# swap357/llama3.np

Measured on AMD Instinct MI355X. Metric: tokens/s stories15M batch-256 seq-256 prefill; % fp32 MFMA peak on FFN GEMM, higher is better.
Workload: dtype fp32; 1 GPU; stories15M prefill, B=256 per GPU x L=256, start_pos 0; global_batch=256, seq_len=256, parallelism=dp1 (batch rows) + RCCL logits gather

## Files before the change

include/llama3hip.h:

```cpp
#ifndef LLAMA3HIP_H
#define LLAMA3HIP_H

#include <stddef.h>
#include <stdint.h>

#ifdef __cplusplus
extern "C" {
#endif

typedef struct l3_ctx l3_ctx;

typedef struct l3_dims {
    int32_t dim;
    int32_t n_layers;
    int32_t n_heads;
    int32_t n_kv_heads;
    int32_t vocab_size;
    int32_t hidden_dim;
    int32_t max_seq_len;
    int32_t max_batch_size;
    float norm_eps;
} l3_dims;

enum l3_weight_kind {
// ... 2 lines not shown
    L3_W_K = 2,
    L3_W_V = 3,
    L3_W_O = 4,
    L3_W_GATE = 5,
    L3_W_UP = 6,
    L3_W_DOWN = 7,
    L3_W_ATTN_NORM = 8,
    L3_W_FFN_NORM = 9,
    L3_W_FINAL_NORM = 10,
    L3_W_LM_HEAD = 11
};

enum l3_kernel_id {
    L3_K_EMBED = 0, L3_K_QKV = 1, L3_K_ATTN = 2, L3_K_OPROJ = 3, L3_K_GATEUP = 4,
    L3_K_DOWN = 5, L3_K_LMHEAD = 6, L3_K_ARGMAX = 7, L3_K_GATHER = 8, L3_K_EMBED_QKV = 9,
    L3_K_FFN = 10, L3_K_COUNT = 11
};

const char* l3_last_error(void);
int l3_device_count(int32_t* n);
int l3_version(int32_t* major, int32_t* minor);
const char* l3_source_hash(void);

int l3_create(int32_t device, const l3_dims* dims, l3_ctx** out);
enum l3_kv_dtype { L3_KV_F32 = 0, L3_KV_BF16 = 1 };
int l3_create_kv(int32_t device, const l3_dims* dims, int32_t kv_dtype, l3_ctx** out);
int l3_kv_info(l3_ctx* ctx, int32_t* dtype, int64_t* bytes);
int l3_destroy(l3_ctx* ctx);
int l3_upload_weight(l3_ctx* ctx, int32_t layer, int32_t kind, const float* host,
                     int64_t rows, int64_t cols);
int l3_finalize(l3_ctx* ctx);
int l3_reset_cache(l3_ctx* ctx);

int l3_forward_host(l3_ctx* ctx, const int64_t* ids_host, int32_t B, int32_t L,
                    int32_t start_pos, float* logits_host);
int l3_set_batch_split(l3_ctx* ctx, int32_t parts, int64_t min_tokens);
int l3_set_last_layer_rows(l3_ctx* ctx, int32_t all_rows);
int l3_set_gemm_x6(l3_ctx* ctx, int32_t on);
int l3_set_weight_bf16(l3_ctx* ctx, int32_t mode);
int l3_weight_bf16_info(l3_ctx* ctx, int32_t* mode, int64_t* bytes, int64_t* gemv_launches);
int l3_set_weight_bf16_rows(l3_ctx* ctx, int32_t max_rows, int64_t min_bytes);
int l3_weight_bf16_rows_info(l3_ctx* ctx, int32_t* max_rows, int64_t* min_bytes, int64_t* launches);
int l3_set_weight_fp8(l3_ctx* ctx, int32_t mode);
int l3_weight_fp8_info(l3_ctx* ctx, int32_t* mode, int64_t* bytes, int64_t* gemv_launches,
                       int64_t* rows_launches);
int l3_set_embed_qkv(l3_ctx* ctx, int32_t on, int64_t max_bytes);
int l3_set_ffn_fused(l3_ctx* ctx, int32_t on);
int l3_forward_dev(l3_ctx* ctx, const int32_t* ids_dev, int32_t B, int32_t L,
                   int32_t start_pos, float* logits_dev);
int l3_score_host(l3_ctx* ctx, const int64_t* ids_host, const int64_t* targets_host, int32_t B, int32_t L,
                  int32_t start_pos, float* logprobs_host, int32_t* argmax_host);
int l3_set_score_workspace(l3_ctx* ctx, int64_t bytes);
int l3_set_sampling(l3_ctx* ctx, float temperature, int32_t top_k, float top_p, uint64_t seed);
int l3_get_sampling(l3_ctx* ctx, float* temperature, int32_t* top_k, float* top_p, uint64_t* seed);
int l3_sample_uniform(uint64_t seed, int32_t row, int32_t pos, float* u);

int l3_greedy_step_host(l3_ctx* ctx, const int64_t* ids_host, int32_t B, int32_t L,
                        int32_t start_pos, int64_t* next_ids_host, float* logits_host);

int l3_greedy_generate_host(l3_ctx* ctx, const int64_t* ids_host, int32_t B, int32_t L,
                            int32_t max_new_tokens, int64_t* out_ids_host);
// ... 225 lines not shown
```

llama3.np_amd/csrc/attention.hip:

```cpp
#include "attn_kernel.h"

namespace l3 {

static void report(AttnRoute* rt, int kernel, int HD, int QBW, int G, int KT, dim3 grid) {
    if (rt) *rt = AttnRoute{kernel, HD, QBW, G, KT, {(int)grid.x, (int)grid.y, (int)grid.z}};
}

template <int HD, int QBW, int G, int KT>
static hipError_t launch(const AttnArgs& a, hipStream_t s, AttnRoute* rt) {
    constexpr int QW = 16 * QBW * (4 / G);
    dim3 grid((a.L + QW - 1) / QW, a.H / G, a.B), block(256);
    report(rt, ATTN_PREFILL, HD, QBW, G, KT, grid);
    hipLaunchKernelGGL((attn_fwd_kernel<HD, QBW, G, KT, true>), grid, block, 0, s, a);
    return hipGetLastError();
}

template <int HD, int KT, int QBIG, int G>
static hipError_t launch_g(const AttnArgs& a, hipStream_t s, AttnRoute* rt) {
    constexpr int WPH = 4 / G;
    if (a.L <= 16 * WPH) return launch<HD, 1, G, KT>(a, s, rt);
    if (QBIG > 2 && a.L <= 32 * WPH) return launch<HD, 2, G, KT>(a, s, rt);
    return launch<HD, QBIG, G, KT>(a, s, rt);
}

template <int HD, int KT, int QBIG>
static hipError_t launch_hd(const AttnArgs& a, hipStream_t s, AttnRoute* rt) {
    const int n_rep = a.H / a.KVH;
    if (n_rep % 4 == 0) return launch_g<HD, KT, QBIG, 4>(a, s, rt);
    if (n_rep % 2 == 0) return launch_g<HD, KT, QBIG, 2>(a, s, rt);
    return launch_g<HD, KT, QBIG, 1>(a, s, rt);
}

template <int HD>
static hipError_t launch_decode(const AttnArgs& a, hipStream_t s, AttnRoute* rt) {
    constexpr int R = 256 / (HD / 4);
    const size_t lds = ((size_t)R * HD + a.Smax) * 4;
    if (a.wo) {
        if (!a.parts || a.D <= 0 || a.D % 4) return hipErrorInvalidValue;
        const dim3 grid(a.H, a.B, (a.D + 63) / 64);
        report(rt, ATTN_DECODE_OPROJ, HD, 0, 0, 0, grid);
        hipLaunchKernelGGL((attn_decode_kernel<HD, true>), grid, dim3(256), lds, s, a);
    } else {
        const dim3 grid(a.H, a.B);
        report(rt, ATTN_DECODE, HD, 0, 0, 0, grid);
        hipLaunchKernelGGL((attn_decode_kernel<HD, false>), grid, dim3(256), lds, s, a);
// ... 45 lines not shown
            case 128: return launch_decode<128>(a, s, rt);
            default: return hipErrorInvalidValue;
        }
    }
    switch (a.HD) {
        case 16: return launch_hd<16, 64, 4>(a, s, rt);
        case 32: return launch_hd<32, 64, 4>(a, s, rt);
        case 48: return launch_hd<48, 64, 4>(a, s, rt);
        case 64: return launch_hd<64, 64, 4>(a, s, rt);
        case 96: return launch_hd<96, 32, 1>(a, s, rt);
        case 128: return launch_hd<128, 32, 1>(a, s, rt);
        default: return hipErrorInvalidValue;
    }
}

hipError_t dcheck_collect_attention(unsigned* out) { return dcheck_collect(out); }

}
```

llama3.np_amd/csrc/attn_kernel.h:

```cpp
#pragma once
#include <type_traits>

#include "kernels.h"

namespace l3 {

typedef float f32x4 __attribute__((ext_vector_type(4)));

template <int HD, int QBW, int G, int KT, bool PK = false>
__global__ void __launch_bounds__(256, 2) attn_fwd_kernel(AttnArgs p) {
    static_assert(HD % 16 == 0 && KT % 16 == 0 && (G == 1 || G == 2 || G == 4), "shape");
    constexpr int WPH = 4 / G;
    constexpr int NQB = QBW * WPH;
    constexpr int QW = 16 * NQB;
    constexpr int ND = HD / 16;
    constexpr int KSTR = HD + 8;
    constexpr int VSTR = HD + 4;
    constexpr int K_F4 = KT * HD / 4;
    constexpr int K_IT = (K_F4 + 255) / 256;
    constexpr int KG = KT / 16;

    __shared__ __attribute__((aligned(16))) float Ks[2][KT][KSTR];
    __shared__ __attribute__((aligned(16))) float Vs[2][KT][VSTR];

// ... 5 lines not shown
    const int qdim = p.H * HD;
    const int fq = lane & 15;
    const int fk = 4 * (lane >> 4);

    int qblk[QBW];
#pragma unroll
    for (int j = 0; j < QBW; ++j)
        qblk[j] = (j & 1) ? (2 * WPH * (j >> 1) + 2 * WPH - 1 - part) : (2 * WPH * (j >> 1) + part);

    const int start_pos = start_of(p);
    const int q_lo = p.q_first + qt * QW;
    const int q_hi = min(p.L, q_lo + QW);
    const int key_end = start_pos + q_hi;
    const int ntiles = (key_end + KT - 1) / KT;
    if (threadIdx.x == 0) L3_DCHECK(start_pos >= 0 && start_pos + p.L <= p.Smax, CHK_ATTN_KEYS);

    f32x4 qreg[QBW][ND];
    f32x4 o[QBW][ND];
    float m_run[QBW], l_run[QBW];
#pragma unroll
    for (int j = 0; j < QBW; ++j) {
        const int ql = min(q_lo + qblk[j] * 16 + fq, p.L - 1);
        const float* src = p.q + ((int64_t)b * p.L + ql) * qdim + h * HD + fk;
#pragma unroll
        for (int dg = 0; dg < ND; ++dg) {
            qreg[j][dg] = *reinterpret_cast<const f32x4*>(src + dg * 16);
            o[j][dg] = f32x4{0.f, 0.f, 0.f, 0.f};
        }
        m_run[j] = -INFINITY;
        l_run[j] = 0.f;
    }

    const int64_t kv_base = ((int64_t)b * p.KVH + kvh) * p.Smax;
    f32x4 rk[K_IT], rv[K_IT];
    auto gload = [&](int tile) {
#pragma unroll
        for (int i = 0; i < K_IT; ++i) {
            const int f = tid + 256 * i;
            const int row = f / (HD / 4), c = (f % (HD / 4)) * 4;
            const int key = min(tile * KT + row, p.Smax - 1);
            if (K_F4 % 256 == 0 || f < K_F4) {
                rk[i] = *reinterpret_cast<const f32x4*>(p.cache_k + (kv_base + key) * HD + c);
                rv[i] = *reinterpret_cast<const f32x4*>(p.cache_v + (kv_base + key) * HD + c);
            }
        }
    };
    auto sstore = [&](int buf) {
#pragma unroll
        for (int i = 0; i < K_IT; ++i) {
            const int f = tid + 256 * i;
            if (K_F4 % 256 == 0 || f < K_F4) {
                const int row = f / (HD / 4), c = (f % (HD / 4)) * 4;
                *reinterpret_cast<f32x4*>(&Ks[buf][row][c]) = rk[i];
                *reinterpret_cast<f32x4*>(&Vs[buf][row][c]) = rv[i];
            }
        }
    };

    gload(0);
    sstore(0);
    __syncthreads();
    int cur = 0;
    for (int tile = 0; tile < ntiles; ++tile) {
        if (tile + 1 < ntiles) gload(tile + 1);
        const int k0 = tile * KT;
        auto qblock_tile = [&](const int j, const int qblock_first, const int qmax_abs, auto masked_tag) {
            constexpr bool MASKED = decltype(masked_tag)::value;
            const int q_abs = start_pos + qblock_first + fq;
            f32x4 sacc[KG];
            bool live[KG];
#pragma unroll
            for (int kg = 0; kg < KG; ++kg) {
                live[kg] = !MASKED || (k0 + kg * 16) <= qmax_abs;
                sacc[kg] = f32x4{0.f, 0.f, 0.f, 0.f};
            }
// ... 90 lines not shown
                }
                __builtin_amdgcn_sched_group_barrier(0x008, 2, 1);
            }
        };
#pragma unroll
        for (int j = 0; j < QBW; ++j) {
            const int qblock_first = q_lo + qblk[j] * 16;
            if (qblock_first >= p.L) continue;
            const int qmax_abs = start_pos + min(qblock_first + 15, p.L - 1);
            if (k0 > qmax_abs) continue;
            if (k0 + KT - 1 <= start_pos + qblock_first)
                qblock_tile(j, qblock_first, qmax_abs, std::integral_constant<bool, false>{});
            else
                qblock_tile(j, qblock_first, qmax_abs, std::integral_constant<bool, true>{});
        }
        if (tile + 1 < ntiles) sstore(cur ^ 1);
        __syncthreads();
        cur ^= 1;
    }

#pragma unroll
    for (int j = 0; j < QBW; ++j) {
        float l = l_run[j];
        l = sum_xor16_32(l);
        const int ql = q_lo + qblk[j] * 16 + fq;
        if (ql < p.L) {
            const float inv = 1.0f / l;
            float* dst = p.out + ((int64_t)b * p.L + ql) * qdim + h * HD + fk;
#pragma unroll
            for (int dg = 0; dg < ND; ++dg)
                *reinterpret_cast<f32x4*>(dst + dg * 16) = o[j][dg] * inv;
// ... 96 lines not shown
```

llama3.np_amd/csrc/embed_qkv.h:

```cpp
#pragma once
#include "gemm_kernel.h"

namespace l3 {

__device__ __forceinline__ f32x4 rope_rotate4(const f32x4 v, const float2 c, const float2 s) {
    return f32x4{__builtin_fmaf(v.x, c.x, -(v.y * s.x)), __builtin_fmaf(v.x, s.x, v.y * c.x),
                 __builtin_fmaf(v.z, c.y, -(v.w * s.y)), __builtin_fmaf(v.z, s.y, v.w * c.y)};
}

constexpr int EQ_ROWS = 16;
constexpr int EQ_R = 4;

template <int CPB>
__global__ void __launch_bounds__(256) embed_qkv_kernel(EmbedQkvArgs p) {
    static_assert(CPB == 64 || CPB == 128 || CPB == 256, "whole waves per row group");
    static_assert(EQ_ROWS % EQ_R == 0, "whole passes");
    constexpr int RPB = 256 / CPB;
    const int cq = threadIdx.x % CPB, rsub = threadIdx.x / CPB;
    const int qdim = p.H * p.HD, kvdim = p.KVH * p.HD, qkvn = qdim + 2 * kvdim, nq = qkvn >> 2;
    const int hd2 = p.HD >> 1;
    const int quad = blockIdx.y * CPB + cq;
    const bool active = quad < nq;
    const int col = 4 * min(quad, nq - 1);
    const int sec = col < qdim ? 0 : (col < qdim + kvdim ? 1 : 2);
// ... 48 lines not shown
```

llama3.np_amd/csrc/kernels.h:

```cpp
#pragma once
#include <hip/hip_runtime.h>
#include <stdint.h>
#include <stdlib.h>

namespace l3 {

inline int env_knob(const char* name, int def) {
    const char* e = getenv(name);
    return e && *e ? atoi(e) : def;
}

enum CheckClass : int { CHK_KV_SLOT = 0, CHK_ATTN_KEYS = 1, CHK_TOKEN_ID = 2, CHK_N = 4 };
#ifdef L3_DEVICE_CHECKS
static __device__ unsigned l3_dcheck_counts[CHK_N];
#define L3_DCHECK(cond, cls)                                                      \
    do {                                                                          \
        if (!(cond)) atomicAdd(&::l3::l3_dcheck_counts[(cls)], 1u);               \
    } while (0)
static inline hipError_t dcheck_collect(unsigned* out) {
    unsigned h[CHK_N] = {};
    hipError_t e = hipMemcpyFromSymbol(h, HIP_SYMBOL(l3_dcheck_counts), sizeof h, 0, hipMemcpyDeviceToHost);
    if (e != hipSuccess) return e;
    for (int i = 0; i < CHK_N; ++i) out[i] += h[i];
    const unsigned z[CHK_N] = {};
// ... 248 lines not shown
__device__ __forceinline__ const float* res_at(const GemmArgs& p, int64_t row, int col) {
    return res_row(p, row) + col;
}

struct AttnArgs {
    const float* q;
    int q_first;
    const float* cache_k;
    const float* cache_v;
    float* out;
    int B, L, start_pos, H, KVH, HD, Smax;
    const int* pos_dev;
    const float* wo;
    float* parts;
    int D;
};

template <typename Args>
__device__ __forceinline__ int start_of(const Args& p) {
    return p.pos_dev ? *p.pos_dev : p.start_pos;
}

struct RaggedState {
    int32_t* pos;
    int32_t* cur_id;
    int32_t* finished;
    int32_t* n_out;
    const int32_t* len;
    const int32_t* budget;
    int32_t* out;
// ... 147 lines not shown
};
bool ffn_fused_takes(int64_t M, int D, int FD);
hipError_t launch_ffn_fused(const FfnArgs& a, hipStream_t s);

struct EmbedQkvArgs {
    const float* table;
    const int32_t* ids;
    float* q_out;
    float* cache_k; float* cache_v;
    const float* rope_cos; const float* rope_sin;
    int T, L, start_pos, H, KVH, HD, Smax, VS;
};
hipError_t launch_qkv_table(const GemmArgs& a, hipStream_t s);
hipError_t launch_embed_qkv(const EmbedQkvArgs& a, hipStream_t s);
hipError_t launch_split_planes(const float* w, unsigned short* w3, int64_t rows, int K, hipStream_t s);
enum AttnRouteKernel : int { ATTN_NONE = -1, ATTN_PREFILL = 0, ATTN_DECODE = 1, ATTN_DECODE_OPROJ = 2 };
struct AttnRoute {
    int kernel = ATTN_NONE;
    int HD = 0, QBW = 0, G = 0, KT = 0;
    int grid[3] = {0, 0, 0};
};
hipError_t launch_attention(const AttnArgs& a, hipStream_t s, AttnRoute* route = nullptr);
hipError_t launch_attention_last(const AttnArgs& a, hipStream_t s, AttnRoute* route = nullptr);
hipError_t launch_argmax(const float* logits, int64_t rows, int n, int32_t* out, hipStream_t s,
                         DecState* st = nullptr);
hipError_t launch_argmax_parts(const ArgmaxPart* parts, int nparts, int32_t* out, hipStream_t s,
                               DecState* st = nullptr, int hist_off = 0, int rows = 1);
hipError_t launch_sample(const float* logits, int64_t rows, int n, int32_t* out, const SampleParams* prm,
                         const float* u_dev, int row0, int pos, hipStream_t s, DecState* st = nullptr);
int gemv_store_blocks(const GemmArgs& a);
bool gemm_is_gemv(const GemmArgs& a);
bool gemv_direct(const GemmArgs& a);
bool gemm_takes_bf16(int epi, const GemmArgs& a);
bool gemm_takes_bf16_rows(int epi, const GemmArgs& a);
constexpr int WB_ROWS_MAX = 64;
bool gemm_takes_fp8(int epi, const GemmArgs& a);
bool gemm_takes_fp8_rows(int epi, const GemmArgs& a);
hipError_t launch_to_fp8_rows(float* w, unsigned char* codes, float* scale, int64_t rows, int K, int sel_rows,
// ... 32 lines not shown
```

llama3.np_amd/csrc/runtime.hip:

```cpp
#include <hip/hip_runtime.h>
#include <rccl/rccl.h>
#include <rocprofiler-sdk-roctx/roctx.h>

#include <cmath>
#include <cstdarg>
#include <cstdio>
#include <cstddef>
#include <cstdlib>
#include <cstring>
#include <mutex>
#include <string>
#include <chrono>
#include <deque>
#include <vector>

#include "../../include/llama3hip.h"
#include "kernels.h"

using namespace l3;

static_assert(offsetof(DecState, pos) == 0, "captured kernels read &DecState::pos as pos_dev");

static thread_local std::string g_err;

// ... 61 lines not shown
    int64_t wb_launches = 0;
    static constexpr int WB_ROWS_DEFAULT = 32;
    static constexpr int64_t WB_ROWS_MIN_BYTES_DEFAULT = (int64_t)32 << 20;
    int wb_rows = WB_ROWS_DEFAULT;
    int64_t wb_rows_min_bytes = WB_ROWS_MIN_BYTES_DEFAULT;
    int64_t wb_rows_launches = 0;
    int weight_fp8 = 0;
    unsigned char* lm_headq = nullptr;
    float* lm_heads = nullptr;
    int64_t wq_bytes = 0;
    int64_t wq_launches = 0;
    int64_t wq_rows_launches = 0;
    static constexpr int64_t EMBED_QKV_CAP_DEFAULT = (int64_t)256 << 20;
    bool embed_qkv = true;
    bool ffn_fused = true;
    int64_t embed_qkv_cap = EMBED_QKV_CAP_DEFAULT;
    float* embed_tab = nullptr;
    bool embed_tab_failed = false;
    bool prune_last = true;
    int64_t split_min_tokens = 8192;
    l3_dims d{};
    int kv_dtype = L3_KV_F32;
    int HD = 0, qdim = 0, kvdim = 0, qkvn = 0;
    float* emb = nullptr;
    float* lm_head = nullptr;
    float* final_norm = nullptr;
    float* rope_cos = nullptr;
    float* rope_sin = nullptr;
    std::vector<Layer> layers;
    bool have_emb = false, have_lm = false, have_fnorm = false, finalized = false;
// ... 112 lines not shown
static int set_dev(l3_ctx* c, bool join = true) {
    HIP_TRY(hipSetDevice(c->device));
    if (join) c->gather_tail = false;
    if (join && c->gather_pending) {
        HIP_TRY(hipStreamWaitEvent(c->stream, c->comm_done_ev, 0));
        c->gather_pending = false;
    }
    return 0;
}

static int spec_resolve(l3_ctx* c);

template <typename F>
static int timed_on(l3_ctx* c, int kind, hipStream_t s, F&& launch) {
    Timer* t = nullptr;
    const unsigned bits = kind == L3_K_FFN ? 1u << L3_K_FFN | 1u << L3_K_GATEUP | 1u << L3_K_DOWN : 1u << kind;
    if (c->timing && (c->timing_mask & bits)) {
        if (c->timer_used == c->timers.size()) {
            Timer nt{};
            HIP_TRY(hipEventCreate(&nt.a));
            HIP_TRY(hipEventCreate(&nt.b));
            c->timers.push_back(nt);
        }
        t = &c->timers[c->timer_used++];
        t->kind = kind;
        HIP_TRY(hipEventRecord(t->a, s));
    }
    hipError_t e = launch();
    if (e != hipSuccess) return fail("kernel launch (kind %d) failed: %s", kind, hipGetErrorString(e));
    if (t) HIP_TRY(hipEventRecord(t->b, s));
    return 0;
// ... 5 lines not shown
}

static int harvest_timers(l3_ctx* c) {
    if (!c->timer_used) return 0;
    HIP_TRY(hipStreamSynchronize(c->stream));
    for (size_t i = 0; i < c->timer_used; ++i) {
        float ms = 0.f;
        HIP_TRY(hipEventElapsedTime(&ms, c->timers[i].a, c->timers[i].b));
        c->tot_ms[c->timers[i].kind] += ms;
        c->cnt[c->timers[i].kind] += 1;
        if (c->timers[i].kind == L3_K_FFN) {
            c->tot_ms[L3_K_GATEUP] += (double)ms * 2.0 / 3.0;
            c->tot_ms[L3_K_DOWN] += (double)ms / 3.0;
            c->cnt[L3_K_GATEUP] += 1;
            c->cnt[L3_K_DOWN] += 1;
        }
    }
    c->timer_used = 0;
    return 0;
}

static void dfree(void* p) {
    if (p) (void)hipFree(p);
}

static void drop_decode_graph(l3_ctx* c) {
    if (c->dec_exec) (void)hipGraphExecDestroy(c->dec_exec);
    if (c->dec_graph) (void)hipGraphDestroy(c->dec_graph);
    c->dec_exec = nullptr;
    c->dec_graph = nullptr;
// ... 131 lines not shown
            return fail("l3_create: L3_WEIGHT_BF16 and L3_WEIGHT_FP8 are both set (one compact weight copy per context)");
        }
        if (const char* rw = getenv("L3_WEIGHT_BF16_ROWS"); rw && *rw) {
            char* end = nullptr;
            const long r = strtol(rw, &end, 10);
            if (end != rw && *end == '\0' && (r == 0 || (r >= 2 && r <= WB_ROWS_MAX))) c->wb_rows = (int)r;
        }
        if (const char* mb = getenv("L3_WEIGHT_BF16_MIN_BYTES"); mb && *mb) {
            char* end = nullptr;
            const long long v = strtoll(mb, &end, 10);
            if (end != mb && *end == '\0' && v >= 0) c->wb_rows_min_bytes = v;
        }
    }
    c->embed_qkv = env_knob("L3_EMBED_QKV", 1) != 0;
    c->ffn_fused = env_knob("L3_FFN_FUSED", 1) != 0;
    {
        c->rag_split_mode = env_knob("L3_RAGGED_SPLIT", 0) == 1 ? 1 : 0;
        const int ch = env_knob("L3_RAGGED_SPLIT_CHUNK", 0);
        if (ch >= RAGGED_CHUNK_MIN && ch <= RAGGED_CHUNK_MAX && ch % 64 == 0) c->rag_split_chunk = ch;
    }
    {
        const int n = env_knob("L3_BATCH_SPLIT", c->split);
        c->split = n < 1 ? 1 : n > l3_ctx::MAX_PARTS ? l3_ctx::MAX_PARTS : n;
    }
    c->HD = HD;
    c->qdim = d.n_heads * HD;
    c->kvdim = d.n_kv_heads * HD;
    c->qkvn = c->qdim + 2 * c->kvdim;
    auto bail = [&](int rc) { l3_destroy(c); return rc; };
    if (set_dev(c)) return bail(1);
// ... 249 lines not shown
        (void)hipGetLastError();
        (void)hipFree(tab);
        c->embed_tab_failed = true;
        return false;
    }
    c->embed_tab = tab;
    return true;
}

extern "C" int l3_set_ffn_fused(l3_ctx* c, int32_t on) {
    CHECK_CTX(c);
    c->ffn_fused = on != 0;
    return 0;
}

extern "C" int l3_set_embed_qkv(l3_ctx* c, int32_t on, int64_t max_bytes) {
    CHECK_CTX(c);
    if (set_dev(c)) return 1;
    c->embed_qkv = on != 0;
    if (max_bytes > 0) c->embed_qkv_cap = max_bytes;
    c->embed_tab_failed = false;
    if (c->embed_tab && (!c->embed_qkv || (int64_t)c->d.vocab_size * c->qkvn * 4 > c->embed_qkv_cap)) {
        HIP_TRY(hipStreamSynchronize(c->stream));
        dfree(c->embed_tab);
        c->embed_tab = nullptr;
    }
    return 0;
}

static int group_members(const l3_group* g);
// ... 350 lines not shown
    }
    if (c->bak_capture) g.kv_bak = c->kv_bak + (int64_t)li * KV_BAK_SLOTS * 2 * 8 * c->d.n_kv_heads * c->HD;
    float* skws = s == c->stream ? c->skws : nullptr;
    g.ws = skws; g.ws_cap = c->skws_cap;
    const bool prune = last_rows && L > 1 && !emb_ids && !pos_dev;
    const bool kv_only = prune && T > 256;
    g.W3 = Ly.wqkv3;
    g.Wb = Ly.wqkvb; g.Wq = Ly.wqkvq; g.wq_scale = Ly.wqkvs;
    g.norm_w = Ly.wqkvb || Ly.wqkvq ? Ly.n_attn : nullptr;
    if (kv_only) {
        g.W = Ly.wqkv + (int64_t)c->qdim * D; g.N = 2 * c->kvdim; g.col_base = c->qdim;
        if (g.W3) g.W3 += (int64_t)c->qdim * 3 * D;
        if (g.Wb) g.Wb += (int64_t)c->qdim * D;
        if (g.Wq) { g.Wq += (int64_t)c->qdim * D; g.wq_scale += c->qdim; }
    }
    if (emb_ids && c->embed_qkv && T > 256 && !pos_dev && !c->fold_in && !g.kv_bak && !g.W3 &&
        embed_table(c, s == c->stream)) {
        EmbedQkvArgs e{};
        e.table = c->embed_tab; e.ids = emb_ids; e.q_out = q; e.cache_k = g.cache_k; e.cache_v = g.cache_v;
        e.rope_cos = c->rope_cos; e.rope_sin = c->rope_sin;
        e.T = (int)T; e.L = L; e.start_pos = start_pos; e.H = g.H; e.KVH = g.KVH; e.HD = g.HD; e.Smax = g.Smax;
        e.VS = c->d.vocab_size;
        if (timed_on(c, L3_K_EMBED_QKV, s, [&] { return launch_embed_qkv(e, s); })) return 1;
    } else if (timed_on(c, L3_K_QKV, s, [&] { return gemm(c, EPI_QKV, g, s); })) return 1;
    if (prune) {
        const int D4 = D;
        float* hl = h + (int64_t)(L - 1) * D4;
        AttnArgs a{};
        a.cache_k = Ly.cache_k + cache0; a.cache_v = Ly.cache_v + cache0; a.out = attn;
        a.H = c->d.n_heads; a.KVH = c->d.n_kv_heads; a.HD = c->HD; a.Smax = c->d.max_seq_len;
        GemmArgs o{};
        if (kv_only) {
            GemmArgs gq = g;
            gq.A = hl; gq.lda = (int64_t)L * D4; gq.W = Ly.wqkv; gq.W3 = nullptr; gq.Wb = Ly.wqkvb; gq.Wq = Ly.wqkvq; gq.wq_scale = Ly.wqkvs; gq.N = c->qdim; gq.col_base = 0;
            gq.M = B; gq.L = 1; gq.start_pos = start_pos + L - 1; gq.force_skinny = gq.split_rows = true;
            gq.ws = nullptr;
            if (timed_on(c, L3_K_QKV, s, [&] { return gemm(c, EPI_QKV, gq, s); })) return 1;
            a.q = q; a.B = B; a.L = 1; a.start_pos = start_pos + L - 1;
// ... 22 lines not shown
    gu.M = (int)T; gu.N = 2 * FD; gu.K = D; gu.norm = true;
    gu.Wb = Ly.wgub; gu.Wq = Ly.wguq; gu.wq_scale = Ly.wgus; gu.norm_w = Ly.wgub || Ly.wguq ? Ly.n_ffn : nullptr;
    gu.eps = c->d.norm_eps;
    GemmArgs dn{};
    dn.A = hid; dn.lda = FD; dn.W = Ly.wd; dn.W3 = Ly.wd3; dn.C = h; dn.ldc = D;
    dn.M = (int)T; dn.N = D; dn.K = FD; dn.norm = false; dn.Wb = Ly.wdb; dn.Wq = Ly.wdq; dn.wq_scale = Ly.wds;
    gu.ws = dn.ws = skws; gu.ws_cap = dn.ws_cap = c->skws_cap;
    static const bool fuse_env = env_knob("L3_DECODE_FUSE_O", 1) != 0;
    const bool fuse_o = fuse_env && L == 1 && c->oparts && c->hsum && b0 == 0 && T == 1 && D % 4 == 0 && c->HD % 16 == 0 &&
                        c->d.max_seq_len <= 8192 && gemv_direct(gu) && gemv_direct(dn);
    AttnArgs a{};
    a.q = q; a.cache_k = Ly.cache_k + cache0; a.cache_v = Ly.cache_v + cache0; a.out = attn;
    a.B = B; a.L = L; a.start_pos = start_pos; a.H = c->d.n_heads; a.KVH = c->d.n_kv_heads;
    a.HD = c->HD; a.Smax = c->d.max_seq_len; a.pos_dev = pos_dev;
    if (fuse_o) { a.wo = Ly.wo; a.parts = c->oparts; a.D = D; }
    if (timed_on(c, L3_K_ATTN, s, [&] { return launch_attention(a, s); })) return 1;
    if (fuse_o) {
        gu.parts = c->oparts;
        gu.nparts = c->d.n_heads;
        gu.x_out = c->hsum;
        dn.res_src = c->hsum;
        if (emb_ids) { gu.A = c->emb; gu.a_rows = emb_ids; }
    } else {
        GemmArgs o{};
        o.A = attn; o.lda = c->qdim; o.W = Ly.wo; o.W3 = Ly.wo3; o.Wb = Ly.wob; o.Wq = Ly.woq; o.wq_scale = Ly.wos; o.C = h; o.ldc = D;
        o.M = (int)T; o.N = D; o.K = c->qdim; o.norm = false;
        o.ws = skws; o.ws_cap = c->skws_cap;
        if (emb_ids) { o.res_src = c->emb; o.res_rows = emb_ids; }
        if (timed_on(c, L3_K_OPROJ, s, [&] { return gemm(c, EPI_RESID, o, s); })) return 1;
    }
    return ffn_pair(c, gu, dn, s);
// ... 3580 lines not shown
```

llama3.np_amd/l3hip.py:

```python

import ctypes
import os
import re
from typing import List, Optional

import numpy as np

HERE = os.path.dirname(os.path.abspath(__file__))
LIB_PATH = os.environ.get("L3_LIB_PATH") or os.path.join(HERE, "csrc", "libllama3hip.so")
HEADER = os.path.join(os.path.dirname(HERE), "include", "llama3hip.h")

W_EMBED, W_Q, W_K, W_V, W_O, W_GATE, W_UP, W_DOWN = range(8)
W_ATTN_NORM, W_FFN_NORM, W_FINAL_NORM, W_LM_HEAD = 8, 9, 10, 11
KERNELS = ["embed", "qkv", "attn", "oproj", "gateup", "down", "lmhead", "argmax", "gather", "embed_qkv", "ffn"]


class Dims(ctypes.Structure):
    _fields_ = [
        ("dim", ctypes.c_int32),
        ("n_layers", ctypes.c_int32),
        ("n_heads", ctypes.c_int32),
        ("n_kv_heads", ctypes.c_int32),
        ("vocab_size", ctypes.c_int32),
        ("hidden_dim", ctypes.c_int32),
        ("max_seq_len", ctypes.c_int32),
        ("max_batch_size", ctypes.c_int32),
        ("norm_eps", ctypes.c_float),
    ]

# ... 56 lines not shown
    "l3_op_silu_host": (ctypes.c_int, [_P, _P, _I64, _P]),
    "l3_op_rmsnorm_host": (ctypes.c_int, [_P, _P, _P, _I64, _I64, _F, _P]),
    "l3_op_rope_host": (ctypes.c_int, [_P, _P, _I32, _I32, _I32, _I32, _P, _P, _P]),
    "l3_op_ffn_host": (ctypes.c_int, [_P, _P, _I64, _I32, _I32, _P, _P, _P, _P]),
    "l3_op_linear_host": (ctypes.c_int, [_P, _P, _I64, _I32, _I32, _P, _P]),
    "l3_op_linear_logprob_host": (ctypes.c_int, [_P, _P, _I64, _I32, _I32, _P, _P, _P, _P, _P]),
    "l3_dev_alloc": (ctypes.c_int, [_P, _SZ, _P]),
    "l3_dev_free": (ctypes.c_int, [_P, _P]),
    "l3_h2d": (ctypes.c_int, [_P, _P, _P, _SZ]),
    "l3_d2h": (ctypes.c_int, [_P, _P, _P, _SZ]),
    "l3_synchronize": (ctypes.c_int, [_P]),
    "l3_set_batch_split": (ctypes.c_int, [_P, _I32, _I64]),
    "l3_set_gemm_x6": (ctypes.c_int, [_P, _I32]),
    "l3_set_embed_qkv": (ctypes.c_int, [_P, _I32, _I64]),
    "l3_set_ffn_fused": (ctypes.c_int, [_P, _I32]),
    "l3_op_ffn_block_host": (ctypes.c_int, [_P, _P, _I64, _I32, _I32, _P, _P, _P, _I32, _I32, _P]),
    "l3_set_weight_bf16": (ctypes.c_int, [_P, _I32]),
    "l3_weight_bf16_info": (ctypes.c_int, [_P, _P, _P, _P]),
    "l3_set_weight_bf16_rows": (ctypes.c_int, [_P, _I32, _I64]),
    "l3_weight_bf16_rows_info": (ctypes.c_int, [_P, _P, _P, _P]),
    "l3_op_linear_bf16_rows_host": (ctypes.c_int, [_P, _P, _I64, _I32, _I32, _P, _P, _F, _P]),
    "l3_op_to_bf16_host": (ctypes.c_int, [_P, _P, _I64, _P, _P]),
    "l3_set_weight_fp8": (ctypes.c_int, [_P, _I32]),
    "l3_weight_fp8_info": (ctypes.c_int, [_P, _P, _P, _P, _P]),
    "l3_op_to_fp8_rows_host": (ctypes.c_int, [_P, _P, _I64, _I32, _P, _P, _P]),
    "l3_op_linear_fp8_host": (ctypes.c_int, [_P, _P, _I64, _I32, _I32, _P, _P, _P, _F, _P, _P]),
    "l3_op_linear_fp8_rows_host": (ctypes.c_int, [_P, _P, _I64, _I32, _I32, _P, _P, _P, _F, _P, _P]),
    "l3_op_linear_bf16_host": (ctypes.c_int, [_P, _P, _I64, _I32, _I32, _P, _P, _F, _P]),
    "l3_op_gemm_host": (ctypes.c_int, [_P, _P]),
    "l3_op_decode_gemm_host": (ctypes.c_int, [_P, _P]),
# ... 135 lines not shown
    "x6": ("bm", "bn", "bk", "waves", "group_m"),
    "rows_bf16": ("mt", "waves", "nt", "tn"),
    "gemv_fp8": ("rows_per_block", "lanes_per_unit", "nt", "row_blocks"),
    "rows_fp8": ("mt", "waves", "nt", "tn"),
    "none": (),
}


def gemm_sentinel(shape, salt: int = 0) -> np.ndarray:
    n = int(np.prod(shape))
    i = np.arange(n, dtype=np.uint64) + np.uint64(salt) * np.uint64(1000003)
    bits = np.uint32(0x40800000) + ((i * np.uint64(2654435761)) & np.uint64(0x3FFFFF)).astype(np.uint32)
    return bits.view(np.float32).reshape(shape)


ATTN_KERNELS = ["prefill", "decode", "decode_oproj"]


def attn_scale_q(q: np.ndarray, hd: int) -> np.ndarray:
    return np.asarray(q, np.float32) * np.float32(1.4426950408889634 / np.sqrt(float(hd)))


def interleave_gate_up(wg: np.ndarray, wu: np.ndarray) -> np.ndarray:
    hidden, K = wg.shape
    if wu.shape != wg.shape or hidden % 16:
        raise ValueError(f"gate {wg.shape} and up {wu.shape} must be equal with hidden % 16 == 0")
    return np.ascontiguousarray(np.stack([wg.reshape(hidden // 16, 16, K), wu.reshape(hidden // 16, 16, K)],
                                         axis=1).reshape(2 * hidden, K))

_lib: Optional[ctypes.CDLL] = None

# ... 440 lines not shown

    def forward_dev(self, ids_dev: int, B: int, L: int, start_pos: int, logits_dev: int) -> None:
        check(lib().l3_forward_dev(self._h, ids_dev, B, L, start_pos, logits_dev))

    def set_batch_split(self, parts: int, min_tokens: int = 8192) -> None:
        check(lib().l3_set_batch_split(self._h, int(parts), int(min_tokens)))

    def set_last_layer_rows(self, all_rows: bool) -> None:
        check(lib().l3_set_last_layer_rows(self._h, int(bool(all_rows))))

    def set_gemm_x6(self, on: bool) -> None:
        check(lib().l3_set_gemm_x6(self._h, int(bool(on))))

    def set_embed_qkv(self, on: bool, max_bytes: int = 0) -> None:
        check(lib().l3_set_embed_qkv(self._h, int(bool(on)), int(max_bytes)))

    def set_ffn_fused(self, on: bool) -> None:
        check(lib().l3_set_ffn_fused(self._h, int(bool(on))))

    def set_weight_bf16(self, mode: int) -> None:
        check(lib().l3_set_weight_bf16(self._h, int(mode)))

    def weight_bf16_info(self) -> dict:
        m, b, n = ctypes.c_int32(0), ctypes.c_int64(0), ctypes.c_int64(0)
        check(lib().l3_weight_bf16_info(self._h, ctypes.byref(m), ctypes.byref(b), ctypes.byref(n)))
        return {"mode": m.value, "bytes": b.value, "gemv_launches": n.value}

    def set_weight_fp8(self, mode: int) -> None:
        check(lib().l3_set_weight_fp8(self._h, int(mode)))

# ... 692 lines not shown
```

Measured before the change: 11.63 million tokens/s.

## Fuse embedding-table QKV lookup and RoPE into first-layer attention kernel

For the first layer in prefill, the attention kernel now reads Q/K/V straight from the precomputed embedding-QKV table using token ids staged in LDS. It applies RoPE in registers, and the last query-tile block writes K/V into the cache. This removes the separate embed_qkv launch and the round trip of Q through global memory. In exchange, every query-tile block re-gathers K/V rows from the table and recomputes RoPE, and the path only covers small head dims, f32 KV and start_pos 0.

```diff
diff --git a/include/llama3hip.h b/include/llama3hip.h
--- a/include/llama3hip.h
+++ b/include/llama3hip.h
@@ -40,7 +40,7 @@
 enum l3_kernel_id {
     L3_K_EMBED = 0, L3_K_QKV = 1, L3_K_ATTN = 2, L3_K_OPROJ = 3, L3_K_GATEUP = 4,
     L3_K_DOWN = 5, L3_K_LMHEAD = 6, L3_K_ARGMAX = 7, L3_K_GATHER = 8, L3_K_EMBED_QKV = 9,
-    L3_K_FFN = 10, L3_K_COUNT = 11
+    L3_K_FFN = 10, L3_K_EMBED_ATTN = 11, L3_K_COUNT = 12
 };
 
 const char* l3_last_error(void);
@@ -71,6 +71,7 @@
 int l3_weight_fp8_info(l3_ctx* ctx, int32_t* mode, int64_t* bytes, int64_t* gemv_launches,
                        int64_t* rows_launches);
 int l3_set_embed_qkv(l3_ctx* ctx, int32_t on, int64_t max_bytes);
+int l3_set_embed_attn(l3_ctx* ctx, int32_t on);
 int l3_set_ffn_fused(l3_ctx* ctx, int32_t on);
 int l3_forward_dev(l3_ctx* ctx, const int32_t* ids_dev, int32_t B, int32_t L,
                    int32_t start_pos, float* logits_dev);
diff --git a/llama3.np_amd/csrc/attention.hip b/llama3.np_amd/csrc/attention.hip
--- a/llama3.np_amd/csrc/attention.hip
+++ b/llama3.np_amd/csrc/attention.hip
@@ -6,29 +6,38 @@
     if (rt) *rt = AttnRoute{kernel, HD, QBW, G, KT, {(int)grid.x, (int)grid.y, (int)grid.z}};
 }
 
-template <int HD, int QBW, int G, int KT>
+template <int HD, int KT>
+constexpr size_t attn_static_lds() { return (size_t)2 * KT * ((HD + 8) + (HD + 4)) * 4; }
+static size_t embed_ids_lds(const AttnArgs& a) { return ((size_t)a.L * 4 + 15) & ~(size_t)15; }
+
+template <int HD, int QBW, int G, int KT, bool EMBED = false>
 static hipError_t launch(const AttnArgs& a, hipStream_t s, AttnRoute* rt) {
     constexpr int QW = 16 * QBW * (4 / G);
     dim3 grid((a.L + QW - 1) / QW, a.H / G, a.B), block(256);
-    report(rt, ATTN_PREFILL, HD, QBW, G, KT, grid);
-    hipLaunchKernelGGL((attn_fwd_kernel<HD, QBW, G, KT, true>), grid, block, 0, s, a);
+    report(rt, EMBED ? ATTN_PREFILL_EMBED : ATTN_PREFILL, HD, QBW, G, KT, grid);
+    if constexpr (EMBED) {
+        if (a.H / a.KVH != G || attn_static_lds<HD, KT>() + embed_ids_lds(a) > 65536) return hipErrorInvalidValue;
+        hipLaunchKernelGGL((attn_fwd_kernel<HD, QBW, G, KT, true, true>), grid, block, embed_ids_lds(a), s, a);
+    } else {
+        hipLaunchKernelGGL((attn_fwd_kernel<HD, QBW, G, KT, true>), grid, block, 0, s, a);
+    }
     return hipGetLastError();
 }
 
-template <int HD, int KT, int QBIG, int G>
+template <int HD, int KT, int QBIG, int G, bool EMBED = false>
 static hipError_t launch_g(const AttnArgs& a, hipStream_t s, AttnRoute* rt) {
     constexpr int WPH = 4 / G;
-    if (a.L <= 16 * WPH) return launch<HD, 1, G, KT>(a, s, rt);
-    if (QBIG > 2 && a.L <= 32 * WPH) return launch<HD, 2, G, KT>(a, s, rt);
-    return launch<HD, QBIG, G, KT>(a, s, rt);
+    if (a.L <= 16 * WPH) return launch<HD, 1, G, KT, EMBED>(a, s, rt);
+    if (QBIG > 2 && a.L <= 32 * WPH) return launch<HD, 2, G, KT, EMBED>(a, s, rt);
+    return launch<HD, QBIG, G, KT, EMBED>(a, s, rt);
 }
 
-template <int HD, int KT, int QBIG>
+template <int HD, int KT, int QBIG, bool EMBED = false>
 static hipError_t launch_hd(const AttnArgs& a, hipStream_t s, AttnRoute* rt) {
     const int n_rep = a.H / a.KVH;
-    if (n_rep % 4 == 0) return launch_g<HD, KT, QBIG, 4>(a, s, rt);
-    if (n_rep % 2 == 0) return launch_g<HD, KT, QBIG, 2>(a, s, rt);
-    return launch_g<HD, KT, QBIG, 1>(a, s, rt);
+    if (n_rep % 4 == 0) return launch_g<HD, KT, QBIG, 4, EMBED>(a, s, rt);
+    if (n_rep % 2 == 0) return launch_g<HD, KT, QBIG, 2, EMBED>(a, s, rt);
+    return launch_g<HD, KT, QBIG, 1, EMBED>(a, s, rt);
 }
 
 template <int HD>
@@ -104,6 +113,37 @@
     }
 }
 
+static size_t embed_static_lds(int HD) {
+    switch (HD) {
+        case 16: return attn_static_lds<16, 64>();
+        case 32: return attn_static_lds<32, 64>();
+        case 48: return attn_static_lds<48, 64>();
+        default: return 0;
+    }
+}
+
+bool attention_embed_takes(const AttnArgs& a) {
+    if (a.B <= 0 || a.L <= 1 || a.KVH <= 0 || a.H % a.KVH != 0) return false;
+    const int n_rep = a.H / a.KVH;
+    if (n_rep != 1 && n_rep != 2 && n_rep != 4) return false;
+    if (a.start_pos != 0 || a.pos_dev || a.q_first != 0 || a.wo || a.L > a.Smax) return false;
+    if (!a.table || !a.ids || !a.rope_cos || !a.rope_sin || !a.kv_out_k || !a.kv_out_v || !a.out) return false;
+    if (a.VS <= 0 || a.qkvn != (a.H + 2 * a.KVH) * a.HD) return false;
+    const size_t st = embed_static_lds(a.HD);
+    return st != 0 && st + embed_ids_lds(a) <= 65536;
+}
+
+hipError_t launch_attention_embed(const AttnArgs& a, hipStream_t s, AttnRoute* rt) {
+    if (rt) *rt = AttnRoute{};
+    if (!attention_embed_takes(a)) return hipErrorInvalidValue;
+    switch (a.HD) {
+        case 16: return launch_hd<16, 64, 4, true>(a, s, rt);
+        case 32: return launch_hd<32, 64, 4, true>(a, s, rt);
+        case 48: return launch_hd<48, 64, 4, true>(a, s, rt);
+        default: return hipErrorInvalidValue;
+    }
+}
+
 hipError_t dcheck_collect_attention(unsigned* out) { return dcheck_collect(out); }
 
 }
diff --git a/llama3.np_amd/csrc/attn_kernel.h b/llama3.np_amd/csrc/attn_kernel.h
--- a/llama3.np_amd/csrc/attn_kernel.h
+++ b/llama3.np_amd/csrc/attn_kernel.h
@@ -2,12 +2,13 @@
 #include <type_traits>
 
 #include "kernels.h"
+#include "rope.h"
 
 namespace l3 {
 
-typedef float f32x4 __attribute__((ext_vector_type(4)));
-
-template <int HD, int QBW, int G, int KT, bool PK = false>
+extern __shared__ int attn_ids_s[];
+
+template <int HD, int QBW, int G, int KT, bool PK = false, bool EMBED = false>
 __global__ void __launch_bounds__(256, 2) attn_fwd_kernel(AttnArgs p) {
     static_assert(HD % 16 == 0 && KT % 16 == 0 && (G == 1 || G == 2 || G == 4), "shape");
     constexpr int WPH = 4 / G;
@@ -43,6 +44,17 @@
     const int key_end = start_pos + q_hi;
     const int ntiles = (key_end + KT - 1) / KT;
     if (threadIdx.x == 0) L3_DCHECK(start_pos >= 0 && start_pos + p.L <= p.Smax, CHK_ATTN_KEYS);
+    const int kvdim = p.KVH * HD;
+    const bool kv_owner = qt == (int)gridDim.x - 1;
+    if constexpr (EMBED) {
+        if (threadIdx.x == 0) L3_DCHECK(start_pos == 0 && p.q_first == 0 && p.H / p.KVH == G, CHK_ATTN_KEYS);
+        for (int l = tid; l < p.L; l += 256) {
+            const int id = p.ids[(int64_t)b * p.L + l];
+            L3_DCHECK(id >= 0 && id < p.VS, CHK_TOKEN_ID);
+            attn_ids_s[l] = id;
+        }
+        __syncthreads();
+    }
 
     f32x4 qreg[QBW][ND];
     f32x4 o[QBW][ND];
@@ -50,10 +62,16 @@
 #pragma unroll
     for (int j = 0; j < QBW; ++j) {
         const int ql = min(q_lo + qblk[j] * 16 + fq, p.L - 1);
-        const float* src = p.q + ((int64_t)b * p.L + ql) * qdim + h * HD + fk;
+        const float* src = EMBED ? p.table + (int64_t)attn_ids_s[ql] * p.qkvn + h * HD + fk
+                                 : p.q + ((int64_t)b * p.L + ql) * qdim + h * HD + fk;
 #pragma unroll
         for (int dg = 0; dg < ND; ++dg) {
             qreg[j][dg] = *reinterpret_cast<const f32x4*>(src + dg * 16);
+            if constexpr (EMBED) {
+                const int ro = (start_pos + ql) * (HD / 2) + ((dg * 16 + fk) >> 1);
+                qreg[j][dg] = rope_rotate4(qreg[j][dg], *reinterpret_cast<const float2*>(p.rope_cos + ro),
+                                           *reinterpret_cast<const float2*>(p.rope_sin + ro));
+            }
             o[j][dg] = f32x4{0.f, 0.f, 0.f, 0.f};
         }
         m_run[j] = -INFINITY;
@@ -67,27 +85,68 @@
         for (int i = 0; i < K_IT; ++i) {
             const int f = tid + 256 * i;
             const int row = f / (HD / 4), c = (f % (HD / 4)) * 4;
-            const int key = min(tile * KT + row, p.Smax - 1);
-            if (K_F4 % 256 == 0 || f < K_F4) {
-                rk[i] = *reinterpret_cast<const f32x4*>(p.cache_k + (kv_base + key) * HD + c);
-                rv[i] = *reinterpret_cast<const f32x4*>(p.cache_v + (kv_base + key) * HD + c);
+            if constexpr (EMBED) {
+                const int key = min(tile * KT + row, p.L - 1);
+                if (K_F4 % 256 == 0 || f < K_F4) {
+                    const float* trow = p.table + (int64_t)attn_ids_s[key] * p.qkvn + qdim + kvh * HD + c;
+                    rk[i] = *reinterpret_cast<const f32x4*>(trow);
+                    rv[i] = *reinterpret_cast<const f32x4*>(trow + kvdim);
+                }
+            } else {
+                const int key = min(tile * KT + row, p.Smax - 1);
+                if (K_F4 % 256 == 0 || f < K_F4) {
+                    rk[i] = *reinterpret_cast<const f32x4*>(p.cache_k + (kv_base + key) * HD + c);
+                    rv[i] = *reinterpret_cast<const f32x4*>(p.cache_v + (kv_base + key) * HD + c);
+                }
             }
         }
     };
-    auto sstore = [&](int buf) {
+    auto sstore = [&](int buf, [[maybe_unused]] int tile) {
+        [[maybe_unused]] float2 rcs[EMBED ? K_IT : 1], rsn[EMBED ? K_IT : 1];
+        if constexpr (EMBED) {
+#pragma unroll
+            for (int i = 0; i < K_IT; ++i) {
+                const int f = tid + 256 * i;
+                const int row = f / (HD / 4), c = (f % (HD / 4)) * 4;
+                const int ro = (start_pos + min(tile * KT + row, p.L - 1)) * (HD / 2) + (c >> 1);
+                if (K_F4 % 256 == 0 || f < K_F4) {
+                    rcs[i] = *reinterpret_cast<const float2*>(p.rope_cos + ro);
+                    rsn[i] = *reinterpret_cast<const float2*>(p.rope_sin + ro);
+                }
+            }
+        }
 #pragma unroll
         for (int i = 0; i < K_IT; ++i) {
             const int f = tid + 256 * i;
             if (K_F4 % 256 == 0 || f < K_F4) {
                 const int row = f / (HD / 4), c = (f % (HD / 4)) * 4;
+                if constexpr (EMBED) {
+                    rk[i] = rope_rotate4(rk[i], rcs[i], rsn[i]);
+                    rv[i] = rope_rotate4(rv[i], float2{1.f, 1.f}, float2{0.f, 0.f});
+                }
                 *reinterpret_cast<f32x4*>(&Ks[buf][row][c]) = rk[i];
                 *reinterpret_cast<f32x4*>(&Vs[buf][row][c]) = rv[i];
             }
         }
+        if constexpr (EMBED) {
+            if (kv_owner) {
+#pragma unroll
+                for (int i = 0; i < K_IT; ++i) {
+                    const int f = tid + 256 * i;
+                    const int row = f / (HD / 4), c = (f % (HD / 4)) * 4;
+                    const int key = tile * KT + row;
+                    if ((K_F4 % 256 == 0 || f < K_F4) && key < p.L) {
+                        L3_DCHECK(start_pos + key < p.Smax, CHK_KV_SLOT);
+                        *reinterpret_cast<f32x4*>(p.kv_out_k + (kv_base + start_pos + key) * HD + c) = rk[i];
+                        *reinterpret_cast<f32x4*>(p.kv_out_v + (kv_base + start_pos + key) * HD + c) = rv[i];
+                    }
+                }
+            }
+        }
     };
 
     gload(0);
-    sstore(0);
+    sstore(0, 0);
     __syncthreads();
     int cur = 0;
     for (int tile = 0; tile < ntiles; ++tile) {
@@ -208,7 +267,7 @@
             else
                 qblock_tile(j, qblock_first, qmax_abs, std::integral_constant<bool, true>{});
         }
-        if (tile + 1 < ntiles) sstore(cur ^ 1);
+        if (tile + 1 < ntiles) sstore(cur ^ 1, tile + 1);
         __syncthreads();
         cur ^= 1;
     }
diff --git a/llama3.np_amd/csrc/embed_qkv.h b/llama3.np_amd/csrc/embed_qkv.h
--- a/llama3.np_amd/csrc/embed_qkv.h
+++ b/llama3.np_amd/csrc/embed_qkv.h
@@ -1,12 +1,8 @@
 #pragma once
 #include "gemm_kernel.h"
+#include "rope.h"
 
 namespace l3 {
-
-__device__ __forceinline__ f32x4 rope_rotate4(const f32x4 v, const float2 c, const float2 s) {
-    return f32x4{__builtin_fmaf(v.x, c.x, -(v.y * s.x)), __builtin_fmaf(v.x, s.x, v.y * c.x),
-                 __builtin_fmaf(v.z, c.y, -(v.w * s.y)), __builtin_fmaf(v.z, s.y, v.w * c.y)};
-}
 
 constexpr int EQ_ROWS = 16;
 constexpr int EQ_R = 4;
diff --git a/llama3.np_amd/csrc/kernels.h b/llama3.np_amd/csrc/kernels.h
--- a/llama3.np_amd/csrc/kernels.h
+++ b/llama3.np_amd/csrc/kernels.h
@@ -286,6 +286,11 @@
     const float* wo;
     float* parts;
     int D;
+    const float* table;
+    const int32_t* ids;
+    const float* rope_cos; const float* rope_sin;
+    float* kv_out_k; float* kv_out_v;
+    int VS, qkvn;
 };
 
 template <typename Args>
@@ -463,7 +468,8 @@
 hipError_t launch_qkv_table(const GemmArgs& a, hipStream_t s);
 hipError_t launch_embed_qkv(const EmbedQkvArgs& a, hipStream_t s);
 hipError_t launch_split_planes(const float* w, unsigned short* w3, int64_t rows, int K, hipStream_t s);
-enum AttnRouteKernel : int { ATTN_NONE = -1, ATTN_PREFILL = 0, ATTN_DECODE = 1, ATTN_DECODE_OPROJ = 2 };
+enum AttnRouteKernel : int { ATTN_NONE = -1, ATTN_PREFILL = 0, ATTN_DECODE = 1, ATTN_DECODE_OPROJ = 2,
+                             ATTN_PREFILL_EMBED = 3  };
 struct AttnRoute {
     int kernel = ATTN_NONE;
     int HD = 0, QBW = 0, G = 0, KT = 0;
@@ -471,6 +477,8 @@
 };
 hipError_t launch_attention(const AttnArgs& a, hipStream_t s, AttnRoute* route = nullptr);
 hipError_t launch_attention_last(const AttnArgs& a, hipStream_t s, AttnRoute* route = nullptr);
+bool attention_embed_takes(const AttnArgs& a);
+hipError_t launch_attention_embed(const AttnArgs& a, hipStream_t s, AttnRoute* route = nullptr);
 hipError_t launch_argmax(const float* logits, int64_t rows, int n, int32_t* out, hipStream_t s,
                          DecState* st = nullptr);
 hipError_t launch_argmax_parts(const ArgmaxPart* parts, int nparts, int32_t* out, hipStream_t s,
diff --git a/llama3.np_amd/csrc/rope.h b/llama3.np_amd/csrc/rope.h
--- /dev/null
+++ b/llama3.np_amd/csrc/rope.h
@@ -0,0 +1,13 @@
+#pragma once
+#include "kernels.h"
+
+namespace l3 {
+
+typedef float f32x4 __attribute__((ext_vector_type(4)));
+
+__device__ __forceinline__ f32x4 rope_rotate4(const f32x4 v, const float2 c, const float2 s) {
+    return f32x4{__builtin_fmaf(v.x, c.x, -(v.y * s.x)), __builtin_fmaf(v.x, s.x, v.y * c.x),
+                 __builtin_fmaf(v.z, c.y, -(v.w * s.y)), __builtin_fmaf(v.z, s.y, v.w * c.y)};
+}
+
+}
diff --git a/llama3.np_amd/csrc/runtime.hip b/llama3.np_amd/csrc/runtime.hip
--- a/llama3.np_amd/csrc/runtime.hip
+++ b/llama3.np_amd/csrc/runtime.hip
@@ -99,6 +99,7 @@
     static constexpr int64_t EMBED_QKV_CAP_DEFAULT = (int64_t)256 << 20;
     bool embed_qkv = true;
     bool ffn_fused = true;
+    bool embed_attn = true;
     int64_t embed_qkv_cap = EMBED_QKV_CAP_DEFAULT;
     float* embed_tab = nullptr;
     bool embed_tab_failed = false;
@@ -241,7 +242,9 @@
 template <typename F>
 static int timed_on(l3_ctx* c, int kind, hipStream_t s, F&& launch) {
     Timer* t = nullptr;
-    const unsigned bits = kind == L3_K_FFN ? 1u << L3_K_FFN | 1u << L3_K_GATEUP | 1u << L3_K_DOWN : 1u << kind;
+    const unsigned bits = kind == L3_K_FFN          ? 1u << L3_K_FFN | 1u << L3_K_GATEUP | 1u << L3_K_DOWN
+                          : kind == L3_K_EMBED_ATTN ? 1u << L3_K_EMBED_ATTN | 1u << L3_K_ATTN | 1u << L3_K_EMBED_QKV
+                                                    : 1u << kind;
     if (c->timing && (c->timing_mask & bits)) {
         if (c->timer_used == c->timers.size()) {
             Timer nt{};
@@ -277,6 +280,11 @@
             c->tot_ms[L3_K_DOWN] += (double)ms / 3.0;
             c->cnt[L3_K_GATEUP] += 1;
             c->cnt[L3_K_DOWN] += 1;
+        }
+        if (c->timers[i].kind == L3_K_EMBED_ATTN) {
+            c->tot_ms[L3_K_ATTN] += ms;
+            c->cnt[L3_K_ATTN] += 1;
+            c->cnt[L3_K_EMBED_QKV] += 1;
         }
     }
     c->timer_used = 0;
@@ -438,6 +446,7 @@
     }
     c->embed_qkv = env_knob("L3_EMBED_QKV", 1) != 0;
     c->ffn_fused = env_knob("L3_FFN_FUSED", 1) != 0;
+    c->embed_attn = env_knob("L3_EMBED_ATTN", 1) != 0;
     {
         c->rag_split_mode = env_knob("L3_RAGGED_SPLIT", 0) == 1 ? 1 : 0;
         const int ch = env_knob("L3_RAGGED_SPLIT_CHUNK", 0);
@@ -717,6 +726,12 @@
     return 0;
 }
 
+extern "C" int l3_set_embed_attn(l3_ctx* c, int32_t on) {
+    CHECK_CTX(c);
+    c->embed_attn = on != 0;
+    return 0;
+}
+
 extern "C" int l3_set_embed_qkv(l3_ctx* c, int32_t on, int64_t max_bytes) {
     CHECK_CTX(c);
     if (set_dev(c)) return 1;
@@ -1097,14 +1112,24 @@
         if (g.Wb) g.Wb += (int64_t)c->qdim * D;
         if (g.Wq) { g.Wq += (int64_t)c->qdim * D; g.wq_scale += c->qdim; }
     }
+    bool attn_done = false;
     if (emb_ids && c->embed_qkv && T > 256 && !pos_dev && !c->fold_in && !g.kv_bak && !g.W3 &&
         embed_table(c, s == c->stream)) {
-        EmbedQkvArgs e{};
-        e.table = c->embed_tab; e.ids = emb_ids; e.q_out = q; e.cache_k = g.cache_k; e.cache_v = g.cache_v;
-        e.rope_cos = c->rope_cos; e.rope_sin = c->rope_sin;
-        e.T = (int)T; e.L = L; e.start_pos = start_pos; e.H = g.H; e.KVH = g.KVH; e.HD = g.HD; e.Smax = g.Smax;
-        e.VS = c->d.vocab_size;
-        if (timed_on(c, L3_K_EMBED_QKV, s, [&] { return launch_embed_qkv(e, s); })) return 1;
+        AttnArgs fa{};
+        fa.out = attn; fa.B = B; fa.L = L; fa.start_pos = start_pos; fa.H = g.H; fa.KVH = g.KVH; fa.HD = g.HD; fa.Smax = g.Smax;
+        fa.table = c->embed_tab; fa.ids = emb_ids; fa.rope_cos = c->rope_cos; fa.rope_sin = c->rope_sin;
+        fa.kv_out_k = g.cache_k; fa.kv_out_v = g.cache_v; fa.VS = c->d.vocab_size; fa.qkvn = c->qkvn;
+        if (c->embed_attn && !prune && c->kv_dtype == L3_KV_F32 && attention_embed_takes(fa)) {
+            if (timed_on(c, L3_K_EMBED_ATTN, s, [&] { return launch_attention_embed(fa, s); })) return 1;
+            attn_done = true;
+        } else {
+            EmbedQkvArgs e{};
+            e.table = c->embed_tab; e.ids = emb_ids; e.q_out = q; e.cache_k = g.cache_k; e.cache_v = g.cache_v;
+            e.rope_cos = c->rope_cos; e.rope_sin = c->rope_sin;
+            e.T = (int)T; e.L = L; e.start_pos = start_pos; e.H = g.H; e.KVH = g.KVH; e.HD = g.HD; e.Smax = g.Smax;
+            e.VS = c->d.vocab_size;
+            if (timed_on(c, L3_K_EMBED_QKV, s, [&] { return launch_embed_qkv(e, s); })) return 1;
+        }
     } else if (timed_on(c, L3_K_QKV, s, [&] { return gemm(c, EPI_QKV, g, s); })) return 1;
     if (prune) {
         const int D4 = D;
@@ -1157,7 +1182,7 @@
     a.B = B; a.L = L; a.start_pos = start_pos; a.H = c->d.n_heads; a.KVH = c->d.n_kv_heads;
     a.HD = c->HD; a.Smax = c->d.max_seq_len; a.pos_dev = pos_dev;
     if (fuse_o) { a.wo = Ly.wo; a.parts = c->oparts; a.D = D; }
-    if (timed_on(c, L3_K_ATTN, s, [&] { return launch_attention(a, s); })) return 1;
+    if (!attn_done && timed_on(c, L3_K_ATTN, s, [&] { return launch_attention(a, s); })) return 1;
     if (fuse_o) {
         gu.parts = c->oparts;
         gu.nparts = c->d.n_heads;
diff --git a/llama3.np_amd/l3hip.py b/llama3.np_amd/l3hip.py
--- a/llama3.np_amd/l3hip.py
+++ b/llama3.np_amd/l3hip.py
@@ -12,7 +12,7 @@
 
 W_EMBED, W_Q, W_K, W_V, W_O, W_GATE, W_UP, W_DOWN = range(8)
 W_ATTN_NORM, W_FFN_NORM, W_FINAL_NORM, W_LM_HEAD = 8, 9, 10, 11
-KERNELS = ["embed", "qkv", "attn", "oproj", "gateup", "down", "lmhead", "argmax", "gather", "embed_qkv", "ffn"]
+KERNELS = ["embed", "qkv", "attn", "oproj", "gateup", "down", "lmhead", "argmax", "gather", "embed_qkv", "ffn", "embed_attn"]
 
 
 class Dims(ctypes.Structure):
@@ -99,6 +99,7 @@
     "l3_set_gemm_x6": (ctypes.c_int, [_P, _I32]),
     "l3_set_embed_qkv": (ctypes.c_int, [_P, _I32, _I64]),
     "l3_set_ffn_fused": (ctypes.c_int, [_P, _I32]),
+    "l3_set_embed_attn": (ctypes.c_int, [_P, _I32]),
     "l3_op_ffn_block_host": (ctypes.c_int, [_P, _P, _I64, _I32, _I32, _P, _P, _P, _I32, _I32, _P]),
     "l3_set_weight_bf16": (ctypes.c_int, [_P, _I32]),
     "l3_weight_bf16_info": (ctypes.c_int, [_P, _P, _P, _P]),
@@ -264,7 +265,7 @@
     return bits.view(np.float32).reshape(shape)
 
 
-ATTN_KERNELS = ["prefill", "decode", "decode_oproj"]
+ATTN_KERNELS = ["prefill", "decode", "decode_oproj", "prefill_embed"]
 
 
 def attn_scale_q(q: np.ndarray, hd: int) -> np.ndarray:
@@ -735,6 +736,9 @@
 
     def set_embed_qkv(self, on: bool, max_bytes: int = 0) -> None:
         check(lib().l3_set_embed_qkv(self._h, int(bool(on)), int(max_bytes)))
+
+    def set_embed_attn(self, on: bool) -> None:
+        check(lib().l3_set_embed_attn(self._h, int(bool(on))))
 
     def set_ffn_fused(self, on: bool) -> None:
         check(lib().l3_set_ffn_fused(self._h, int(bool(on))))
```

New measurement: 11.71 million tokens/s, median of 6. About the same (+0.7%).
